# smups/rustronomy-watershed

Measured on AMD Instinct MI355X. Metric: Mpixels/s segmenting watershed, 8192x8192 u8, device-resident (throughput, 4 transforms of distinct fields in flight; one transform alone: value_one_transform_alone), higher is better.
Workload: dtype u8 image / u32 stamps+labels (integer min/max/compare); 1 GPU; 8192x8192 u8 uniform[0,254) random field per GPU, segmenting transform, max_water_level 254, seeds = find_local_minima (7320260 on rank 0's first field), engine fused; 4 contexts in flight, each transforming ITS OWN field and seed list (generator seeds 1..4); parallelism=independent fields x1, world_size=1, devices_visible=1, fields_per_gpu=1

## Files before the change

### rustronomy-watershed_amd/csrc/ws_relax.hip

```cpp
#include "ws_common.hpp"
#include "ws_relax_plan.hpp"
#include "ws_relax_patch.hpp"
#include "ws_relax_queue.hpp"

#include <algorithm>
#include <cstdio>
#include <cstdlib>

namespace wsk {

#ifdef WS_DIAG_STAMPS
__device__ unsigned long long *g_diag = nullptr;
#define WS_STAMP(slot)                                                                          \
  do {                                                                                          \
    if (threadIdx.x == 0 && g_diag) g_diag[(size_t)blockIdx.x * 8 + (slot)] = __builtin_amdgcn_s_memrealtime(); \
  } while (0)
#define WS_STAMP_VALUE(slot, v)                                                                 \
  do {                                                                                          \
    if (threadIdx.x == 0 && g_diag) g_diag[(size_t)blockIdx.x * 8 + (slot)] = (v);              \
  } while (0)
#define WS_ACC_DECL unsigned long long ws_acc_t = 0, ws_acc[3] = {0, 0, 0}
#define WS_ACC_T0 (ws_acc_t = __builtin_amdgcn_s_memrealtime())
#define WS_ACC(k) do { const unsigned long long n_ = __builtin_amdgcn_s_memrealtime(); ws_acc[k] += n_ - ws_acc_t; ws_acc_t = n_; } while (0)
#define WS_ACC_STORE do { if (threadIdx.x == 0 && g_diag) { g_diag[(size_t)blockIdx.x * 8 + 5] = ws_acc[0]; g_diag[(size_t)blockIdx.x * 8 + 6] = ws_acc[1]; g_diag[(size_t)blockIdx.x * 8 + 7] = ws_acc[2]; } } while (0)
#else
#define WS_ACC_DECL do {} while (0)
#define WS_ACC_T0 do {} while (0)
#define WS_ACC(k) do {} while (0)
#define WS_ACC_STORE do {} while (0)
#define WS_STAMP(slot) do {} while (0)
#define WS_STAMP_VALUE(slot, v) do {} while (0)
#endif

#ifdef WS_TUNING
#define WS_QPHASE(k) do { if (PERSIST && threadIdx.x == 0) { const unsigned long long n_ = __builtin_amdgcn_s_memrealtime(); q_ph[k] += (uint32_t)(n_ - q_tp); q_tp = n_; } } while (0)
#define WS_QPHASE0 do { if (PERSIST && threadIdx.x == 0) q_tp = __builtin_amdgcn_s_memrealtime(); } while (0)
#else
#define WS_QPHASE(k) do {} while (0)
#define WS_QPHASE0 do {} while (0)
#endif

__device__ __forceinline__ uint32_t plane_or_bit(const uint32_t *src, size_t p, int bits) {
  return bits ? (src[p >> 5] >> (p & 31u)) & 1u : src[p];
}

constexpr uint32_t ST_BORDER = 0x40000000u;
constexpr uint32_t ST_SELF = 0x80000000u;
constexpr uint32_t ST_PASS = 0x3FFFFFFFu;

template <int TW, int TH>
__device__ __forceinline__ unsigned long long relax_todo(int first, int stride, int chunk, int H, int W, int tilesX, int tilesY, int otherX,
                                                         int otherY, int shifted, uint32_t pass,
                                                         const uint32_t *__restrict__ stamps_prev, int read_same = 0) {
  const int lane = threadIdx.x & 63;
  const int ox = shifted ? TW / 2 : 0, oy = shifted ? TH / 2 : 0;
  const int t = first + lane * stride;
  const bool mine = lane < chunk && t < tilesX * tilesY;
  const int tx = mine ? t % tilesX : 0, ty = mine ? t / tilesX : 0;
  bool run = mine && tx * TW - ox < W && ty * TH - oy < H;
  if (read_same) {
    const size_t tt = (size_t)ty * tilesX + tx;
    const uint32_t s0 = stamps_prev[tt * 4];
    bool flagged = (s0 & ST_PASS) == pass && (s0 & ST_SELF) != 0u;
    const int nx[4] = {tx, tx, tx - 1, tx + 1}, ny[4] = {ty - 1, ty + 1, ty, ty};
    const int qa[4] = {2, 0, 1, 0}, qb[4] = {3, 1, 3, 2};
#pragma unroll
    for (int k = 0; k < 4; ++k) {
      const bool ok = nx[k] >= 0 && nx[k] < tilesX && ny[k] >= 0 && ny[k] < tilesY;
      const size_t ot = (size_t)(ok ? ny[k] : 0) * tilesX + (ok ? nx[k] : 0);
      const uint32_t a = stamps_prev[ot * 4 + qa[k]], b = stamps_prev[ot * 4 + qb[k]];
      flagged |= ok && (((a & ST_PASS) == pass && (a & ST_BORDER) != 0u) || ((b & ST_PASS) == pass && (b & ST_BORDER) != 0u));
    }
    run = run && flagged;
  } else if (pass != 0) {
    bool flagged = false;
#pragma unroll
    for (int q = 0; q < 4; ++q) {
      const int qx = q & 1, qy = q >> 1;
      const int oi = tx + qx - (shifted ? 1 : 0), oj = ty + qy - (shifted ? 1 : 0);
      const bool ok = oi >= 0 && oi < otherX && oj >= 0 && oj < otherY;
      const size_t ot = (size_t)(ok ? oj : 0) * otherX + (ok ? oi : 0);
      const uint32_t st = stamps_prev[ot * 4 + (3 - q)];
      flagged |= ok && st == pass;
    }
    run = run && flagged;
  }
  return __builtin_amdgcn_ballot_w64(run);
}


template <bool TRACK, bool RIGHT, int LX>
__device__ __forceinline__ void scan_row(uint32_t (&t)[RX_P], const uint32_t (&b)[RX_P], uint32_t halo_in, int xl, bool &changed) {
  const uint32_t t0 = RIGHT ? t[0] : t[3], t1 = RIGHT ? t[1] : t[2], t2 = RIGHT ? t[2] : t[1], t3 = RIGHT ? t[3] : t[0];
  const uint32_t b0 = RIGHT ? b[0] : b[3], b1 = RIGHT ? b[1] : b[2], b2 = RIGHT ? b[2] : b[1], b3 = RIGHT ? b[3] : b[0];
  uint32_t hi = t0;
  hi = med3u(b1, hi + 1u, t1); hi = med3u(b2, hi + 1u, t2); hi = med3u(b3, hi + 1u, t3);
  uint32_t lo = b0;
  lo = med3u(b1, lo + 1u, t1); lo = med3u(b2, lo + 1u, t2); lo = med3u(b3, lo + 1u, t3);
  const uint32_t bias = RIGHT ? (uint32_t)(RX_P * (LX - 1 - xl)) : (uint32_t)(RX_P * xl);
  lo += bias;
  hi += bias;
  auto combine = [&](uint32_t plo, uint32_t phi) {
    const uint32_t nlo = med3u(lo, plo, hi), nhi = med3u(lo, phi, hi);
    lo = nlo; hi = nhi;
  };
#define WS_DPP(old, v, ctrl, rows) (uint32_t)__builtin_amdgcn_update_dpp((int)(old), (int)(v), ctrl, rows, 0xF, false)
  if (RIGHT) {
    combine(WS_DPP(0u, lo, 0x111, 0xF), WS_DPP(~0u, hi, 0x111, 0xF));
    combine(WS_DPP(0u, lo, 0x112, 0xF), WS_DPP(~0u, hi, 0x112, 0xF));
    combine(WS_DPP(0u, lo, 0x114, 0xF), WS_DPP(~0u, hi, 0x114, 0xF));
    combine(WS_DPP(0u, lo, 0x118, 0xF), WS_DPP(~0u, hi, 0x118, 0xF));
    combine(WS_DPP(0u, lo, 0x142, 0xA), WS_DPP(~0u, hi, 0x142, 0xA));
    if (LX == 64) combine(WS_DPP(0u, lo, 0x143, 0xC), WS_DPP(~0u, hi, 0x143, 0xC));
  } else {
    combine(WS_DPP(0u, lo, 0x101, 0xF), WS_DPP(~0u, hi, 0x101, 0xF));
    combine(WS_DPP(0u, lo, 0x102, 0xF), WS_DPP(~0u, hi, 0x102, 0xF));
    combine(WS_DPP(0u, lo, 0x104, 0xF), WS_DPP(~0u, hi, 0x104, 0xF));
    combine(WS_DPP(0u, lo, 0x108, 0xF), WS_DPP(~0u, hi, 0x108, 0xF));
    {
      const int lane = (int)(threadIdx.x & 63u);
      const uint32_t l16 = (uint32_t)__builtin_amdgcn_readlane((int)lo, 16), h16 = (uint32_t)__builtin_amdgcn_readlane((int)hi, 16);
      const uint32_t l48 = (uint32_t)__builtin_amdgcn_readlane((int)lo, 48), h48 = (uint32_t)__builtin_amdgcn_readlane((int)hi, 48);
      const bool r0 = lane < 16, r2 = lane >= 32 && lane < 48;
      combine(r0 ? l16 : (r2 ? l48 : 0u), r0 ? h16 : (r2 ? h48 : ~0u));
      if (LX == 64) {
        const uint32_t l32 = (uint32_t)__builtin_amdgcn_readlane((int)lo, 32), h32 = (uint32_t)__builtin_amdgcn_readlane((int)hi, 32);
        combine(lane < 32 ? l32 : 0u, lane < 32 ? h32 : ~0u);
      }
    }
  }
#undef WS_DPP
  const uint32_t leaves = med3u(lo, halo_in + (uint32_t)(RX_P * LX), hi) - bias;
  uint32_t vin = RIGHT ? lane_left(halo_in, leaves) : lane_right(halo_in, leaves);
  if (LX != 64) vin = (RIGHT ? xl == 0 : xl == LX - 1) ? halo_in : vin;
  const uint32_t n0 = med3u(b0, vin + 1u, t0), n1 = med3u(b1, n0 + 1u, t1), n2 = med3u(b2, n1 + 1u, t2), n3 = med3u(b3, n2 + 1u, t3);
  if (TRACK) changed |= (n0 != t0) | (n1 != t1) | (n2 != t2) | (n3 != t3);
  t[RIGHT ? 0 : 3] = n0; t[RIGHT ? 1 : 2] = n1; t[RIGHT ? 2 : 1] = n2; t[RIGHT ? 3 : 0] = n3;
}

template <int NB, int TW, bool SPLIT>
__device__ __forceinline__ void scan_cols_both(patch_t &T, const patch_t &B, uint32_t *fn, const uint32_t *halo_top, const uint32_t *halo_bottom,
                                               int band, int xl) {
  auto slot = [&](int dir, int k, int which) { return fn + (((size_t)dir * NB + k) * 2 + which) * TW + xl * RX_P; };
  {
    uint32_t lo[RX_P], hi[RX_P];
#pragma unroll
    for (int dir = 0; dir < 2; ++dir) {
#pragma unroll
      for (int c = 0; c < RX_P; ++c) {
        uint32_t h = T[dir ? 3 : 0][c], l = B[dir ? 3 : 0][c];
#pragma unroll
        for (int k = 1; k < RX_P; ++k) {
          const int r = dir ? RX_P - 1 - k : k;
          h = med3u(B[r][c], h + 1u, T[r][c]);
          l = med3u(B[r][c], l + 1u, T[r][c]);
        }
        lo[c] = l; hi[c] = h;
      }
      *reinterpret_cast<u32x4_t *>(slot(dir, band, 0)) = u32x4_t{lo[0], lo[1], lo[2], lo[3]};
      *reinterpret_cast<u32x4_t *>(slot(dir, band, 1)) = u32x4_t{hi[0], hi[1], hi[2], hi[3]};
// ... 513 lines not shown
      const size_t t = (size_t)tile_y * tilesX + tile_x;
      if (!CHUNKED && chunk == 3 && (ed & 32u)) const_cast<uint32_t *>(stamps_prev)[((size_t)tile_y * otherX + tile_x + 1) * 4 + 2] = pass + 2;
      if (write_same) {
        if (ed & 33u) stamps_cur[t * 4 + 0] = (pass + 1) | (ed & 1u ? ST_BORDER : 0u) | (ed & 32u ? ST_SELF : 0u);
        if (ed & 2u) stamps_cur[t * 4 + 1] = (pass + 1) | ST_BORDER;
        if (ed & 4u) stamps_cur[t * 4 + 2] = (pass + 1) | ST_BORDER;
        if (ed & 8u) stamps_cur[t * 4 + 3] = (pass + 1) | ST_BORDER;
      } else {
        if (ed & 1u) stamps_cur[t * 4 + 0] = pass + 1;
        if (ed & 2u) stamps_cur[t * 4 + 1] = pass + 1;
        if (ed & 4u) stamps_cur[t * 4 + 2] = pass + 1;
        if (ed & 8u) stamps_cur[t * 4 + 3] = pass + 1;
      }
      if (ed & 47u) pf.edge_changed[(pass % COUNTER_RING) * FLAG_SLOT + stripe] = 1u;
      if (append_next) {
        const bool want[5] = {(ed & 32u) != 0u, (ed & 64u) != 0u && tile_y > 0, (ed & 128u) != 0u && tile_y + 1 < tilesY,
                              (ed & 256u) != 0u && tile_x > 0, (ed & 512u) != 0u && tile_x + 1 < tilesX};
        const uint32_t who[5] = {(uint32_t)t, (uint32_t)(t - tilesX), (uint32_t)(t + tilesX), (uint32_t)(t - 1), (uint32_t)(t + 1)};
        uint32_t n = s_ncand;
        if (PERSIST == 2) {
          uint32_t bk[5];
          bk[0] = s_qbucket;
#pragma unroll
          for (int k = 1; k < 5; ++k) {
            bk[k] = min(s_sidemin[k - 1] >> q.pq_shift, (uint32_t)(PQ_B - 1));
            if (want[k]) bk[0] = min(bk[0], bk[k]);
          }
#pragma unroll
          for (int k = 0; k < 5; ++k)
            if (want[k]) s_cand[n++] = who[k] | (bk[k] << 24);
        } else {
#pragma unroll
          for (int k = 0; k < 5; ++k)
            if (want[k]) s_cand[n++] = who[k];
        }
        s_ncand = n;
      }
      pf.any_change[stripe] = 1u;
    }
    count_tile_run(pf, stripe, (uint32_t)(TW * TH / 2048), iters);
  }
  WS_STAMP(3);
  WS_QPHASE(2);
  if (PERSIST == 2) {
    queue_hand_in_flood_order(q, (uint32_t)tile, tid, lane, use_list, s_cand, s_ncand, s_qtile, s_qbucket, s_handoff);
    WS_QPHASE(3);
    continue;
  }
  if (PERSIST) {
    queue_hand_in_first_come(q, (uint32_t)tile, tid, lane, s_cand, s_ncand);
    WS_QPHASE(3);
    continue;
  }
  if (!CHUNKED) break;
  if (use_list) {
    entry = s_next[runs_done & 1u];
    ++runs_done;
    const bool last = entry >= n_entries;
    if (append_next && tid < 64 && (last || s_ncand > RX_CAND - 5u)) append_flush(tile_list, list_cap, pass, s_cand, s_ncand);
    if (last) break;
  } else {
    todo &= todo - 1;
    if (todo == 0) break;
  }
  }
}

template <int TW, int TH>
__global__ __launch_bounds__(256) void k_relax_list(int H, int W, int tilesX, int tilesY, int otherX, int otherY, int shifted,
                                                    uint32_t pass, const uint32_t *__restrict__ stamps_prev, uint32_t *tile_list,
                                                    int read_same, uint32_t list_cap) {
  const int lane = threadIdx.x & 63;
  const int first = (int)((blockIdx.x * blockDim.x + threadIdx.x) & ~63u);
  if ((uint32_t)(first + lane) <= list_cap) tile_list[RL_HDR + 2 * (size_t)list_cap + first + lane] = 0u;
  const unsigned long long todo = relax_todo<TW, TH>(first, 1, 64, H, W, tilesX, tilesY, otherX, otherY, shifted, pass, stamps_prev, read_same);
  if (todo == 0) return;
  uint32_t base = 0;
  if (lane == 0) base = atomicAdd(&tile_list[pass & 3u], (uint32_t)__popcll(todo));
  base = __shfl(base, 0, 64);
  if ((todo >> lane) & 1ull)
    tile_list[RL_HDR + (pass & 1u) * (size_t)list_cap + base + __popcll(todo & ((1ull << lane) - 1ull))] = (uint32_t)(first + lane);
}

template <int TW, int TH, int OTW, int OTH>
__global__ __launch_bounds__(256) void k_relax_list_regrid(int H, int W, int tilesX, int tilesY, int oldX, int oldY, uint32_t pass,
                                                           const uint32_t *__restrict__ stamps_prev, uint32_t *tile_list, uint32_t list_cap,
                                                           int persist) {
  const int lane = threadIdx.x & 63;
  const int first = (int)((blockIdx.x * blockDim.x + threadIdx.x) & ~63u);
  const int t = first + lane;
  bool run = false;
  if (t < tilesX * tilesY) {
    const int tx = t % tilesX, ty = t / tilesX;
    const int x_lo = max(tx * TW - 1, 0) / OTW, x_hi = min((tx * TW + TW) / OTW, oldX - 1);
    const int y_lo = max(ty * TH - 1, 0) / OTH, y_hi = min((ty * TH + TH) / OTH, oldY - 1);
    for (int oy = y_lo; oy <= y_hi; ++oy)
      for (int ox = x_lo; ox <= x_hi; ++ox) {
        const uint4 st = *reinterpret_cast<const uint4 *>(stamps_prev + ((size_t)oy * oldX + ox) * 4);
        run |= (st.x & ST_PASS) == pass || (st.y & ST_PASS) == pass || (st.z & ST_PASS) == pass || (st.w & ST_PASS) == pass;
      }
    run = run && tx * TW < W && ty * TH < H;
  }
  if ((uint32_t)t <= list_cap) tile_list[RL_HDR + 2 * (size_t)list_cap + t] = persist && run ? 1u : 0u;
  const unsigned long long todo = __builtin_amdgcn_ballot_w64(run);
  if (todo == 0) return;
  uint32_t base = 0;
  if (lane == 0) {
    base = atomicAdd(&tile_list[persist ? RLQ_TAIL : (pass & 3u)], (uint32_t)__popcll(todo));
    if (persist) atomicAdd(&tile_list[RLQ_PENDING], (uint32_t)__popcll(todo));
  }
  base = __shfl(base, 0, 64);
  const uint32_t idx = base + (uint32_t)__popcll(todo & ((1ull << lane) - 1ull));
  if (persist == 2) {
    uint32_t *avail = tile_list + pq_base(list_cap);
    if (lane == 0) atomicAdd(avail, (uint32_t)__popcll(todo));
    if ((lane & 31) == 0) (avail + PQ_HDR)[(first >> 5) + (lane >> 5)] = (uint32_t)(todo >> (lane & 32));
  } else if (run && persist) reinterpret_cast<unsigned long long *>(tile_list + RL_HDR)[idx] = ((unsigned long long)(idx + 1u) << 32) | (uint32_t)t;
  else if (run) tile_list[RL_HDR + (pass & 1u) * (size_t)list_cap + idx] = (uint32_t)t;
}

template <int TW, int TH>
__global__ __launch_bounds__(256) void k_relax_list_all(int H, int W, int tilesX, int tilesY, uint32_t pass, uint32_t *tile_list, uint32_t list_cap) {
  const int t = blockIdx.x * blockDim.x + threadIdx.x;
  if (t == 0) { tile_list[pass & 3u] = (uint32_t)(tilesX * tilesY); tile_list[4 + (pass & 3u)] = 0u; }
  if ((uint32_t)t <= list_cap) tile_list[RL_HDR + 2 * (size_t)list_cap + t] = 0u;
  if (t < tilesX * tilesY) tile_list[RL_HDR + (pass & 1u) * (size_t)list_cap + t] = (uint32_t)t;
}

size_t relax_list_words(int h, int w) {
  const uint32_t tiles = (uint32_t)relax_tiles(h, w);
  return pq_base(tiles) + PQ_HDR + (size_t)PQ_B * pq_words_per_bucket(tiles);
}

size_t relax_tiles(int h, int w) { return relax_plan_tiles(h, w); }

__global__ void k_flag_tile_rows(uint32_t *prev, int sx, int bottom_row, uint32_t pass, int halo_flags) {
  const int i = blockIdx.x * blockDim.x + threadIdx.x;
  if (i >= sx * 4) return;
  if (halo_flags & 1) prev[i] = pass;
  if (halo_flags & 2) prev[(size_t)bottom_row * sx * 4 + i] = pass;
}

hipError_t block_flag_border_tiles(hipStream_t s, uint32_t *stamps, int h, int w, uint32_t pass, int halo_flags) {
  if ((pass & 1u) != 0 || h == 0 || w == 0) return hipErrorInvalidValue;
  const int th = RX_NW * RX_P;
  const int sx = (w + RX_TW - 1) / RX_TW + 1;
  const size_t cap = relax_tiles(h, w) * 4;
  const int bottom_row = (h - 2) / th + 1;
  k_flag_tile_rows<<<(sx * 4 + 255) / 256, 256, 0, s>>>(stamps + cap, sx, bottom_row, pass, halo_flags);
  return hipGetLastError();
}


__global__ __launch_bounds__(64 * RX_NW, 4) void k_relax0_tall(const uint8_t *__restrict__ img, uint32_t stride32, uint32_t *keys, int H, int W,
                                                               int tilesX, int flagAX, int flagSX, uint32_t max_level, uint32_t *stamps_own,
                                                               uint32_t *stamps_rerun, PassFlags pf, uint32_t max_iters,
                                                               const uint32_t *__restrict__ seed_mask, int SH, int check_carry, uint32_t *tile_list) {
  constexpr int NB = RX_NW, TW = RX_TW, TH = RX0_TH;
  constexpr uint32_t pass = 0;
  __shared__ __attribute__((aligned(16))) uint32_t sRow[2 * NB + 2][TW];
  __shared__ uint32_t s_flag[3];

  launch_prologue(pf, tile_list, pass);
  const int tile = (int)xcd_span_index(blockIdx.x, gridDim.x);
  const int tile_x = tile % tilesX, tile_y = tile / tilesX;
  const int x0 = tile_x * TW, y0 = tile_y * TH;
  if (x0 >= W || y0 >= H) return;
  const int tid = threadIdx.x, lane = tid & 63, band = tid >> 6;
  const int gx0 = x0 + lane * RX_P, gyb = y0 + band * RX0_PH;
  if (tid == 0) { s_flag[0] = 0; s_flag[1] = 0; s_flag[2] = 0; }

  uint32_t T[RX0_PH][RX_P], B[RX0_PH][RX_P];
  uint32_t Lh[RX0_PH], Rh[RX0_PH];
  const bool dims24 = (uint32_t)W < (1u << 24) && (uint32_t)H < (1u << 24);
  const uint32_t gxc0 = (uint32_t)min(gx0, W - RX_P);
  const int xh_raw = lane < 32 ? x0 - 1 : x0 + TW;
  const uint32_t xh = (uint32_t)min(max(xh_raw, 0), W - 1);
  const bool xh_ok = lane < 32 ? x0 > 0 : x0 + TW < W;
  const int gy_halo_raw = band == 0 ? y0 - 1 : y0 + TH;
  const uint32_t gy_halo = (uint32_t)min(max(gy_halo_raw, 0), H - 1);
  u32x4_t halo_row;
  {
    uint32_t iv[RX0_PH];
#pragma unroll
    for (int r = 0; r < RX0_PH; ++r) {
      const uint32_t gyc = (uint32_t)min(gyb + r, H - 1);
      const uint32_t ro = dims24 ? __umul24(gyc, (uint32_t)W) : gyc * (uint32_t)W;
      const uint32_t p = ro + gxc0, ph_ = ro + xh;
      const uint32_t nib = seed_mask[p >> 5] >> (p & 31u);
      iv[r] = *reinterpret_cast<const uint32_t *>(img + ((unsigned long long)gyc * stride32 + gxc0));
      Lh[r] = (seed_mask[ph_ >> 5] >> (ph_ & 31u)) & 1u;
      T[r][0] = nib & 1u; T[r][1] = nib & 2u; T[r][2] = nib & 4u; T[r][3] = nib & 8u;
    }
    const uint32_t p = (dims24 ? __umul24(gy_halo, (uint32_t)W) : gy_halo * (uint32_t)W) + gxc0;
    const uint32_t nib = seed_mask[p >> 5] >> (p & 31u);
    halo_row = u32x4_t{nib & 1u, nib & 2u, nib & 4u, nib & 8u};
    patch_bases(iv, B, max_level);
  }
  halo_row = seed_stamps(T, Lh, halo_row);
  const bool inner = SH == H && x0 >= 1 && x0 + TW <= W - 1 && y0 >= 1 && y0 + TH <= H - 1;
  if (!inner) {
    int ry = SH == H ? gyb : gyb % SH;
#pragma unroll
    for (int r = 0; r < RX0_PH; ++r) {
      const int gy = gyb + r;
      const bool row_ok = gy < H, row_int = ry >= 1 && ry < SH - 1 && gy < H;
#pragma unroll
      for (int c = 0; c < RX_P; ++c) {
        const int gx = gx0 + c;
        if (!(row_ok && gx < W)) T[r][c] = KEY_INF;
        if (!(row_int && gx >= 1 && gx < W - 1)) B[r][c] = KEY_INF;
      }
      if (!(row_ok && xh_ok)) Lh[r] = KEY_INF;
      if (++ry == SH) ry = 0;
    }
    const bool ok = gy_halo_raw >= 0 && gy_halo_raw < H;
    if (!(ok && gx0 + 0 < W)) halo_row.x = KEY_INF;
    if (!(ok && gx0 + 1 < W)) halo_row.y = KEY_INF;
    if (!(ok && gx0 + 2 < W)) halo_row.z = KEY_INF;
    if (!(ok && gx0 + 3 < W)) halo_row.w = KEY_INF;
  }
#pragma unroll
  for (int r = 0; r < RX0_PH; ++r) {
#pragma unroll
    for (int c = 0; c < RX_P; ++c) B[r][c] = min(B[r][c], T[r][c]);
    Rh[r] = Lh[r];
  }
  auto refresh_columns = [&]() {
#pragma unroll
    for (int r = 0; r < RX0_PH; ++r) {
      Lh[r] = lane_left(Lh[r], T[r][3]);
      Rh[r] = lane_right(Rh[r], T[r][0]);
    }
  };
  auto publish_rows = [&]() {
    *reinterpret_cast<u32x4_t *>(&sRow[1 + 2 * band][lane * RX_P]) = u32x4_t{T[0][0], T[0][1], T[0][2], T[0][3]};
    *reinterpret_cast<u32x4_t *>(&sRow[2 + 2 * band][lane * RX_P]) = u32x4_t{T[RX0_PH - 1][0], T[RX0_PH - 1][1], T[RX0_PH - 1][2], T[RX0_PH - 1][3]};
  };
  if (band == 0) *reinterpret_cast<u32x4_t *>(&sRow[0][lane * RX_P]) = halo_row;
  if (band == NB - 1) *reinterpret_cast<u32x4_t *>(&sRow[2 * NB + 1][lane * RX_P]) = halo_row;
  publish_rows();
  __syncthreads();

  uint32_t iters = 0;
  bool unfinished = max_iters == 0;
  uint32_t up[RX_P], dn[RX_P];
  auto fetch_rows = [&]() {
    const u32x4_t up4 = *reinterpret_cast<const u32x4_t *>(&sRow[2 * band][lane * RX_P]);
    const u32x4_t dn4 = *reinterpret_cast<const u32x4_t *>(&sRow[2 * band + 3][lane * RX_P]);
    up[0] = up4.x; up[1] = up4.y; up[2] = up4.z; up[3] = up4.w;
    dn[0] = dn4.x; dn[1] = dn4.y; dn[2] = dn4.z; dn[3] = dn4.w;
  };
  for (; max_iters != 0;) {
    ++iters;
    {
      bool untracked = false;
      fetch_rows();
      if (iters == 1) {
        refresh_columns();
        sweep_rows<false, true>(T, B, up, dn, Lh, Rh, untracked);
        refresh_columns();
        sweep_cols<false, true>(T, B, up, dn, Lh, Rh, untracked);
      }
      refresh_columns();
      sweep_rows<false, false>(T, B, up, dn, Lh, Rh, untracked);
      publish_rows();
      __syncthreads();
    }
    bool changed = false;
    fetch_rows();
    refresh_columns();
    sweep_cols<true, false>(T, B, up, dn, Lh, Rh, changed);
    const uint32_t slot = (iters - 1) % 3;
    if (__builtin_amdgcn_ballot_w64(changed) != 0) {
      publish_rows();
      if (lane == 0) s_flag[slot] = 1;
    }
    __syncthreads();
    const bool again = s_flag[slot] != 0;
    if (tid == 0) s_flag[(slot + 2) % 3] = 0;
    if (!again) break;
    if (iters >= max_iters) { unfinished = true; break; }
  }
  WS_STAMP(0);
  WS_STAMP_VALUE(4, iters);

  uint32_t ovf = 0;
  if (gx0 < W) {
#pragma unroll
    for (int r = 0; r < RX0_PH; ++r) {
      const int gy = gyb + r;
      if (gy < H) *reinterpret_cast<u32x4_t *>(keys + (size_t)gy * W + gx0) = u32x4_t{T[r][0], T[r][1], T[r][2], T[r][3]};
      if (check_carry) {
#pragma unroll
        for (int c = 0; c < RX_P; ++c)
          ovf |= (T[r][c] != 0u && T[r][c] < KEY_INF && ((T[r][c] + 1u) & RING_MASK) <= 1u);
      }
    }
  }
  if (ovf) atomicExch(pf.overflow, 1u);
  const uint32_t stripe = (blockIdx.x % NSTRIPE) * STRIPE_STRIDE;
  bool edge = false;
  if (band == 0) {
    const u32x4_t a = *reinterpret_cast<const u32x4_t *>(&sRow[0][lane * RX_P]);
    edge |= matters(0u, T[0][0], a.x) || matters(0u, T[0][1], a.y) || matters(0u, T[0][2], a.z) || matters(0u, T[0][3], a.w);
  }
  if (band == NB - 1) {
    const u32x4_t a = *reinterpret_cast<const u32x4_t *>(&sRow[2 * NB + 1][lane * RX_P]);
    constexpr int l = RX0_PH - 1;
    edge |= matters(0u, T[l][0], a.x) || matters(0u, T[l][1], a.y) || matters(0u, T[l][2], a.z) || matters(0u, T[l][3], a.w);
  }
  if (lane == 0 || lane == 63) {
#pragma unroll
    for (int r = 0; r < RX0_PH; ++r) edge |= matters(0u, T[r][lane == 0 ? 0 : 3], lane == 0 ? Lh[r] : Rh[r]);
  }
  if (edge) pf.edge_changed[(pass % COUNTER_RING) * FLAG_SLOT + stripe] = 1u;
  if (tid == 0) {
    if (unfinished) {
#pragma unroll
      for (int k = 0; k < RX0_TH / (RX_NW * RX_P); ++k) {
        const int fy = tile_y * (RX0_TH / (RX_NW * RX_P)) + k;
        if (fy * (RX_NW * RX_P) >= H) break;
        stamps_rerun[((size_t)fy * flagSX + tile_x + 1) * 4 + 2] = pass + 2;
        uint32_t *own = stamps_own + ((size_t)fy * flagAX + tile_x) * 4;
        own[0] = pass + 1; own[1] = pass + 1; own[2] = pass + 1; own[3] = pass + 1;
      }
      pf.edge_changed[(pass % COUNTER_RING) * FLAG_SLOT + stripe] = 1u;
    }
    pf.any_change[stripe] = 1u;
    count_tile_run(pf, stripe, (uint32_t)(TW * TH / 2048), 2u * iters);
  }
}

__global__ __launch_bounds__(64 * RX_NW, 4) void k_relax_strips_tall(const uint8_t *__restrict__ img, uint32_t stride32, uint32_t *keys, int H, int W,
                                                                     int stripsX, int flagSX, uint32_t max_level, uint32_t pass, uint32_t *stamps_cur,
                                                                     PassFlags pf, uint32_t max_iters, int SH, int check_carry, uint32_t *tile_list) {
  constexpr int NB = RX_NW, TW = RX_TW, TH = RX0_TH;
  __shared__ __attribute__((aligned(16))) uint32_t sRow[2 * NB + 2][TW];
  __shared__ __attribute__((aligned(16))) uint32_t sInitRow[2][TW];
  __shared__ uint32_t s_flag[3];
  __shared__ uint32_t s_edges;
  __shared__ uint64_t s_sum[64 * NB];
  __shared__ uint32_t sInitCol[RX0_PH][64 * NB];

  launch_prologue(pf, tile_list, pass);
  const int tile = (int)xcd_span_index(blockIdx.x, gridDim.x);
  const int tile_x = tile % stripsX, tile_y = tile / stripsX;
  const int y0 = tile_y * TH;
  if (y0 >= H || (tile_x * 32 + 1) * SEAM_PX >= W) return;
  const int tid = threadIdx.x, lane = tid & 63, band = tid >> 6;
  const int seam_x = (tile_x * 32 + (lane >> 1) + 1) * SEAM_PX;
  const bool has_seam = seam_x < W;
  const int fx = seam_x / SEAM_PX - 1 + (lane & 1);
  {
    bool settled = true;
#pragma unroll
    for (int k = 0; k < TH / SEAM_PY; ++k) {
      const int fy = tile_y * (TH / SEAM_PY) + k;
      const bool there = has_seam && fy * SEAM_PY < H;
      const uint32_t word = stamps_cur[there ? ((size_t)fy * flagSX + fx + 1) * 4 + 2 : 2];
      settled &= !there || word == pass + 1;
    }
    if (__builtin_amdgcn_ballot_w64(settled) == ~0ull) return;
  }
  const int gx0 = has_seam ? seam_x - RX_P + (lane & 1) * RX_P : W, gyb = y0 + band * RX0_PH;
  if (tid == 0) { s_edges = 0; s_flag[0] = 0; s_flag[1] = 0; s_flag[2] = 0; }

  uint32_t T[RX0_PH][RX_P], B[RX0_PH][RX_P];
  uint32_t halo[RX0_PH];
  const uint32_t gxc0 = (uint32_t)min(gx0, W - RX_P);
  const int xh_raw = (lane & 1) ? gx0 + RX_P : gx0 - 1;
  const uint32_t xh = (uint32_t)min(max(xh_raw, 0), W - 1);
  const bool xh_ok = has_seam && xh_raw < W;
  const int gy_halo_raw = band == 0 ? y0 - 1 : y0 + TH;
  const uint32_t gy_halo = (uint32_t)min(max(gy_halo_raw, 0), H - 1);
  u32x4_t halo_row;
  {
    u32x4_t kv[RX0_PH];
    uint32_t iv[RX0_PH];
#pragma unroll
    for (int r = 0; r < RX0_PH; ++r) {
      const uint32_t gyc = (uint32_t)min(gyb + r, H - 1);
      iv[r] = *reinterpret_cast<const uint32_t *>(img + ((unsigned long long)gyc * stride32 + gxc0));
      kv[r] = *reinterpret_cast<const u32x4_t *>(keys + (size_t)gyc * W + gxc0);
      halo[r] = keys[(size_t)gyc * W + xh];
    }
    halo_row = *reinterpret_cast<const u32x4_t *>(keys + (size_t)gy_halo * W + gxc0);
#pragma unroll
    for (int r = 0; r < RX0_PH; ++r) { T[r][0] = kv[r].x; T[r][1] = kv[r].y; T[r][2] = kv[r].z; T[r][3] = kv[r].w; }
    patch_bases(iv, B, max_level);
  }
  {
    int ry = SH == H ? gyb : gyb % SH;
#pragma unroll
    for (int r = 0; r < RX0_PH; ++r) {
      const int gy = gyb + r;
      const bool row_ok = gy < H, row_int = ry >= 1 && ry < SH - 1 && gy < H;
#pragma unroll
      for (int c = 0; c < RX_P; ++c) {
        const int gx = gx0 + c;
        if (!(row_ok && gx < W)) T[r][c] = KEY_INF;
        if (!(row_int && gx >= 1 && gx < W - 1)) B[r][c] = KEY_INF;
      }
      if (!(row_ok && xh_ok)) halo[r] = KEY_INF;
      if (++ry == SH) ry = 0;
    }
    const bool ok = gy_halo_raw >= 0 && gy_halo_raw < H;
    if (!(ok && gx0 + 0 < W)) halo_row.x = KEY_INF;
    if (!(ok && gx0 + 1 < W)) halo_row.y = KEY_INF;
    if (!(ok && gx0 + 2 < W)) halo_row.z = KEY_INF;
    if (!(ok && gx0 + 3 < W)) halo_row.w = KEY_INF;
  }
  uint32_t Lh[RX0_PH], Rh[RX0_PH];
  {
    uint64_t sum_before = 0;
#pragma unroll
    for (int r = 0; r < RX0_PH; ++r) {
#pragma unroll
      for (int c = 0; c < RX_P; ++c) {
        B[r][c] = min(B[r][c], T[r][c]);
        sum_before += T[r][c];
      }
      Lh[r] = halo[r];
      Rh[r] = halo[r];
      sInitCol[r][tid] = (lane & 1) ? T[r][RX_P - 1] : T[r][0];
    }
    s_sum[tid] = sum_before;
  }
  auto refresh_columns = [&]() {
#pragma unroll
    for (int r = 0; r < RX0_PH; ++r) {
      Lh[r] = lane_left(Lh[r], T[r][RX_P - 1]);
      Rh[r] = lane_right(Rh[r], T[r][0]);
      Lh[r] = (lane & 1) ? Lh[r] : halo[r];
      Rh[r] = (lane & 1) ? halo[r] : Rh[r];
// ... 260 lines not shown
```

Measured before the change: 184,800 Mpixels/s.

## Track per-row dirty masks in pass-0 relax and sweep only rows needing work

```diff
diff --git a/rustronomy-watershed_amd/csrc/ws_pass0_rows.hpp b/rustronomy-watershed_amd/csrc/ws_pass0_rows.hpp
--- /dev/null
+++ b/rustronomy-watershed_amd/csrc/ws_pass0_rows.hpp
@@ -0,0 +1,25 @@
+#pragma once
+
+#include <stdint.h>
+
+#if defined(__HIPCC__)
+#define P0R_FN __host__ __device__ static inline
+#else
+#define P0R_FN static inline
+#endif
+
+#define P0R_ROWS 8
+#define P0R_ALL 0xFFu
+
+P0R_FN uint32_t p0r_after_round1(uint32_t changed) { return (changed | (changed << 1) | (changed >> 1)) & P0R_ALL; }
+
+P0R_FN uint32_t p0r_wake(uint32_t need, int above_changed, int below_changed) {
+  return need | (above_changed ? 1u : 0u) | (below_changed ? 1u << (P0R_ROWS - 1) : 0u);
+}
+
+P0R_FN uint32_t p0r_row_swept(uint32_t need, int r, int changed) {
+  return changed ? (need | ((7u << r) >> 1)) & P0R_ALL : need & ~(1u << r);
+}
+
+P0R_FN uint32_t p0r_later_half_rounds(uint32_t max_rounds) { return max_rounds == 0 ? 0u : 2u * (max_rounds - 1u); }
+P0R_FN uint32_t p0r_rounds(uint32_t half_rounds) { return 1u + (half_rounds + 1u) / 2u; }
diff --git a/rustronomy-watershed_amd/csrc/ws_relax.hip b/rustronomy-watershed_amd/csrc/ws_relax.hip
--- a/rustronomy-watershed_amd/csrc/ws_relax.hip
+++ b/rustronomy-watershed_amd/csrc/ws_relax.hip
@@ -2,10 +2,12 @@
 #include "ws_relax_plan.hpp"
 #include "ws_relax_patch.hpp"
 #include "ws_relax_queue.hpp"
+#include "ws_pass0_rows.hpp"
 
 #include <algorithm>
 #include <cstdio>
 #include <cstdlib>
+#include <type_traits>
 
 namespace wsk {
 
@@ -825,6 +827,52 @@
 }
 
 
+constexpr int ICMP_NE = 33, ICMP_ULT = 36;
+__device__ __forceinline__ void sweep_left_by_row(uint32_t (&T)[RX0_PH][RX_P], const uint32_t (&B)[RX0_PH][RX_P], const uint32_t (&up)[RX_P],
+                                                  const uint32_t (&dn)[RX_P], const uint32_t (&L)[RX0_PH], const uint32_t (&R)[RX0_PH],
+                                                  uint64_t (&changed)[RX0_PH]) {
+#pragma unroll
+  for (int c = RX_P - 1; c >= 0; --c)
+#pragma unroll
+    for (int r = 0; r < RX0_PH; ++r) {
+      const uint32_t u = r == 0 ? up[c] : T[r - 1][c], d = r == RX0_PH - 1 ? dn[c] : T[r + 1][c];
+      const uint32_t l = c == 0 ? L[r] : T[r][c - 1], rt = c == RX_P - 1 ? R[r] : T[r][c + 1];
+      const uint32_t n = med3u(B[r][c], min(min(u, d), min(l, rt)) + 1u, T[r][c]);
+      changed[r] |= __builtin_amdgcn_uicmp(n, T[r][c], ICMP_NE);
+      T[r][c] = n;
+    }
+}
+
+template <int r, bool LTR>
+__device__ __forceinline__ bool sweep_needed_row(uint32_t (&T)[RX0_PH][RX_P], const uint32_t (&B)[RX0_PH][RX_P], const u32x4_t *above,
+                                                 const u32x4_t *below, uint32_t (&L)[RX0_PH], uint32_t (&R)[RX0_PH], uint32_t &need) {
+  need = __builtin_amdgcn_readfirstlane(need);
+  asm("" : "+s"(need));
+  if ((need & (1u << r)) == 0) return false;
+  uint32_t out[RX_P] = {0u, 0u, 0u, 0u};
+  if (r == 0 || r == RX0_PH - 1) {
+    const u32x4_t o = r == 0 ? *above : *below;
+    out[0] = o.x; out[1] = o.y; out[2] = o.z; out[3] = o.w;
+  }
+  L[r] = lane_left(L[r], T[r][RX_P - 1]);
+  R[r] = lane_right(R[r], T[r][0]);
+  const uint32_t left = L[r], right = R[r];
+  __builtin_amdgcn_sched_barrier(0);
+  uint64_t ch = 0;
+#pragma unroll
+  for (int k = 0; k < RX_P; ++k) {
+    const int c = LTR ? k : RX_P - 1 - k;
+    const uint32_t u = r == 0 ? out[c] : T[r - 1][c], d = r == RX0_PH - 1 ? out[c] : T[r + 1][c];
+    const uint32_t l = c == 0 ? left : T[r][c - 1], rt = c == RX_P - 1 ? right : T[r][c + 1];
+    const uint32_t m = max(B[r][c], min(min(u, d), min(l, rt)) + 1u);
+    ch |= __builtin_amdgcn_uicmp(m, T[r][c], ICMP_ULT);
+    __builtin_amdgcn_sched_barrier(0);
+    T[r][c] = min(T[r][c], m);
+  }
+  need = p0r_row_swept(need, r, ch != 0);
+  return ch != 0;
+}
+
 __global__ __launch_bounds__(64 * RX_NW, 4) void k_relax0_tall(const uint8_t *__restrict__ img, uint32_t stride32, uint32_t *keys, int H, int W,
                                                                int tilesX, int flagAX, int flagSX, uint32_t max_level, uint32_t *stamps_own,
                                                                uint32_t *stamps_rerun, PassFlags pf, uint32_t max_iters,
@@ -833,6 +881,7 @@
   constexpr uint32_t pass = 0;
   __shared__ __attribute__((aligned(16))) uint32_t sRow[2 * NB + 2][TW];
   __shared__ uint32_t s_flag[3];
+  __shared__ uint32_t s_edge[3][2][NB + 2];
 
   launch_prologue(pf, tile_list, pass);
   const int tile = (int)xcd_span_index(blockIdx.x, gridDim.x);
@@ -842,6 +891,7 @@
   const int tid = threadIdx.x, lane = tid & 63, band = tid >> 6;
   const int gx0 = x0 + lane * RX_P, gyb = y0 + band * RX0_PH;
   if (tid == 0) { s_flag[0] = 0; s_flag[1] = 0; s_flag[2] = 0; }
+  if (tid < 3 * 2 * (NB + 2)) (&s_edge[0][0][0])[tid] = 0;
 
   uint32_t T[RX0_PH][RX_P], B[RX0_PH][RX_P];
   uint32_t Lh[RX0_PH], Rh[RX0_PH];
@@ -917,43 +967,94 @@
 
   uint32_t iters = 0;
   bool unfinished = max_iters == 0;
-  uint32_t up[RX_P], dn[RX_P];
-  auto fetch_rows = [&]() {
-    const u32x4_t up4 = *reinterpret_cast<const u32x4_t *>(&sRow[2 * band][lane * RX_P]);
-    const u32x4_t dn4 = *reinterpret_cast<const u32x4_t *>(&sRow[2 * band + 3][lane * RX_P]);
-    up[0] = up4.x; up[1] = up4.y; up[2] = up4.z; up[3] = up4.w;
-    dn[0] = dn4.x; dn[1] = dn4.y; dn[2] = dn4.z; dn[3] = dn4.w;
+  auto publish_first = [&]() {
+    *reinterpret_cast<u32x4_t *>(&sRow[1 + 2 * band][lane * RX_P]) = u32x4_t{T[0][0], T[0][1], T[0][2], T[0][3]};
   };
-  for (; max_iters != 0;) {
-    ++iters;
+  auto publish_last = [&]() {
+    *reinterpret_cast<u32x4_t *>(&sRow[2 + 2 * band][lane * RX_P]) = u32x4_t{T[RX0_PH - 1][0], T[RX0_PH - 1][1], T[RX0_PH - 1][2], T[RX0_PH - 1][3]};
+  };
+  const u32x4_t *const above = reinterpret_cast<const u32x4_t *>(&sRow[2 * band][lane * RX_P]);
+  const u32x4_t *const below = reinterpret_cast<const u32x4_t *>(&sRow[2 * band + 3][lane * RX_P]);
+  const int wband = __builtin_amdgcn_readfirstlane(band);
+  uint32_t need = 0;
+  if (max_iters != 0) {
     {
+      uint32_t up[RX_P], dn[RX_P];
+      auto fetch_rows = [&]() {
+        const u32x4_t up4 = *above, dn4 = *below;
+        up[0] = up4.x; up[1] = up4.y; up[2] = up4.z; up[3] = up4.w;
+        dn[0] = dn4.x; dn[1] = dn4.y; dn[2] = dn4.z; dn[3] = dn4.w;
+      };
       bool untracked = false;
       fetch_rows();
-      if (iters == 1) {
-        refresh_columns();
-        sweep_rows<false, true>(T, B, up, dn, Lh, Rh, untracked);
-        refresh_columns();
-        sweep_cols<false, true>(T, B, up, dn, Lh, Rh, untracked);
-      }
+      refresh_columns();
+      sweep_rows<false, true>(T, B, up, dn, Lh, Rh, untracked);
+      refresh_columns();
+      sweep_cols<false, true>(T, B, up, dn, Lh, Rh, untracked);
       refresh_columns();
       sweep_rows<false, false>(T, B, up, dn, Lh, Rh, untracked);
       publish_rows();
       __syncthreads();
-    }
-    bool changed = false;
-    fetch_rows();
-    refresh_columns();
-    sweep_cols<true, false>(T, B, up, dn, Lh, Rh, changed);
-    const uint32_t slot = (iters - 1) % 3;
-    if (__builtin_amdgcn_ballot_w64(changed) != 0) {
-      publish_rows();
-      if (lane == 0) s_flag[slot] = 1;
+      uint64_t ch[RX0_PH];
+#pragma unroll
+      for (int r = 0; r < RX0_PH; ++r) ch[r] = 0;
+      fetch_rows();
+      refresh_columns();
+      sweep_left_by_row(T, B, up, dn, Lh, Rh, ch);
+      uint32_t changed = 0;
+#pragma unroll
+      for (int r = 0; r < RX0_PH; ++r) changed |= ch[r] != 0 ? 1u << r : 0u;
+      need = p0r_after_round1(changed);
+      if (changed & 1u) { publish_first(); if (lane == 0) s_edge[0][0][wband + 1] = 1; }
+      if (changed >> (RX0_PH - 1)) { publish_last(); if (lane == 0) s_edge[0][1][wband + 1] = 1; }
+      if (need != 0 && lane == 0) s_flag[0] = 1;
     }
     __syncthreads();
-    const bool again = s_flag[slot] != 0;
-    if (tid == 0) s_flag[(slot + 2) % 3] = 0;
-    if (!again) break;
-    if (iters >= max_iters) { unfinished = true; break; }
+    bool again = __builtin_amdgcn_readfirstlane(s_flag[0]) != 0;
+    uint32_t hr = 0, k = 0;
+    auto half_round = [&](auto upward_tag) -> bool {
+      constexpr bool UPWARD = decltype(upward_tag)::value;
+      ++k;
+      const uint32_t slot = k % 3, prev = (k + 2) % 3;
+      need = p0r_wake(need, __builtin_amdgcn_readfirstlane(s_edge[prev][1][wband]) != 0,
+                      __builtin_amdgcn_readfirstlane(s_edge[prev][0][wband + 2]) != 0);
+      bool first, last;
+      if (UPWARD) {
+        last = sweep_needed_row<7, true>(T, B, above, below, Lh, Rh, need);
+        sweep_needed_row<6, true>(T, B, above, below, Lh, Rh, need);
+        sweep_needed_row<5, true>(T, B, above, below, Lh, Rh, need);
+        sweep_needed_row<4, true>(T, B, above, below, Lh, Rh, need);
+        sweep_needed_row<3, true>(T, B, above, below, Lh, Rh, need);
+        sweep_needed_row<2, true>(T, B, above, below, Lh, Rh, need);
+        sweep_needed_row<1, true>(T, B, above, below, Lh, Rh, need);
+        first = sweep_needed_row<0, true>(T, B, above, below, Lh, Rh, need);
+      } else {
+        first = sweep_needed_row<0, false>(T, B, above, below, Lh, Rh, need);
+        sweep_needed_row<1, false>(T, B, above, below, Lh, Rh, need);
+        sweep_needed_row<2, false>(T, B, above, below, Lh, Rh, need);
+        sweep_needed_row<3, false>(T, B, above, below, Lh, Rh, need);
+        sweep_needed_row<4, false>(T, B, above, below, Lh, Rh, need);
+        sweep_needed_row<5, false>(T, B, above, below, Lh, Rh, need);
+        sweep_needed_row<6, false>(T, B, above, below, Lh, Rh, need);
+        last = sweep_needed_row<7, false>(T, B, above, below, Lh, Rh, need);
+      }
+      if (first) { publish_first(); if (lane == 0) s_edge[slot][0][wband + 1] = 1; }
+      if (last) { publish_last(); if (lane == 0) s_edge[slot][1][wband + 1] = 1; }
+      if (need != 0 && lane == 0) s_flag[slot] = 1;
+      __syncthreads();
+      if (tid == 0) s_flag[prev] = 0;
+      if (lane == 0) { s_edge[prev][0][wband + 1] = 0; s_edge[prev][1][wband + 1] = 0; }
+      return __builtin_amdgcn_readfirstlane(s_flag[slot]) != 0;
+    };
+    const uint32_t hr_cap = p0r_later_half_rounds(max_iters);
+    while (again) {
+      if (hr == hr_cap) { unfinished = true; break; }
+      const bool after_up = half_round(std::true_type{});
+      const bool after_down = half_round(std::false_type{});
+      hr += after_up ? 2u : 1u;
+      again = after_up && after_down;
+    }
+    iters = p0r_rounds(hr);
   }
   WS_STAMP(0);
   WS_STAMP_VALUE(4, iters);
```

After: 182,900 Mpixels/s. About the same (-1.0%).
